# Alfredu/dislib

Measured on AMD Instinct MI355X. Metric: KMeans samples·iters/sec at 1/2/4/8 GPUs + % of HBM/MFMA roofline, higher is better.
Workload: dtype f64

## Files before the change

### dislib_amd/csrc/dkm_dense.h

```cpp
#pragma once

#include <hip/hip_runtime.h>

#include "dkm_internal.h"

namespace dkm {

constexpr int BLOCK = 256;
constexpr size_t LDS_BUDGET = 80 * 1024;
constexpr size_t LDS_PER_CU = 160 * 1024;

enum : int { AM_NONE = 0, AM_ON = 1, AM_DELTA = 2, AM_INLDS = 4,
             AM_MLIST = 8 };
__host__ __device__ __forceinline__ bool am_full(int m) {
  return (m & (AM_ON | AM_DELTA)) == AM_ON;
}

struct DevInfo {
  int cus = 256;
};
DevInfo dev_info();
int resident_blocks(const void *kf, int block, size_t lds);

template <class TX>
__device__ __forceinline__ double ld_x(const TX *p) {
  return (double)(*p);
}

__host__ __device__ __forceinline__ int lds_stride(int d) {
  return (d & 1) ? d : d + 1;
}
__host__ __device__ __forceinline__ int64_t lds_acc_len(int64_t k, int d) {
  return k * lds_stride(d) + k;
}

__device__ __forceinline__ void lds_add(double *p, double v) {
  __hip_atomic_fetch_add(p, v, __ATOMIC_RELAXED, __HIP_MEMORY_SCOPE_WORKGROUP);
}

struct AccTarget {
  double *rows;
  double *cnt;
  int stride;
  bool lds;
  __device__ __forceinline__ void add(int row, int t, double v) const {
    double *p = rows + (int64_t)row * stride + t;
    if (lds)
      lds_add(p, v);
    else
      atomic_add_f64(p, v);
  }
  __device__ __forceinline__ void count(int row, double v) const {
    if (lds)
      lds_add(cnt + row, v);
    else
      atomic_add_f64(cnt + row, v);
  }
};

__device__ __forceinline__ AccTarget acc_target(int amode, double *lds_acc,
                                                double *acc, int64_t k,
                                                int d) {
  if (amode & AM_INLDS) {
    const int ds = lds_stride(d);
    return AccTarget{lds_acc, lds_acc + k * ds, ds, true};
  }
  return AccTarget{acc, acc + k * d, d, false};
}

__device__ __forceinline__ void zero_lds_acc(double *lds_acc, int64_t k,
                                             int d) {
  const int64_t len = lds_acc_len(k, d);
  for (int64_t e = threadIdx.x; e < len; e += blockDim.x) lds_acc[e] = 0.0;
}

__device__ __forceinline__ void flush_lds_acc(const double *lds_acc,
                                              double *acc, int64_t k, int d) {
  const int ds = lds_stride(d);
  const int64_t kd = k * d;
  for (int64_t e = threadIdx.x; e < kd + k; e += blockDim.x) {
    const double v = e < kd ? lds_acc[(e / d) * ds + (e % d)]
                            : lds_acc[k * ds + (e - kd)];
    if (v != 0.0) atomic_add_f64(acc + e, v);
  }
}

template <bool VEC, class TX>
__device__ __forceinline__ void load8(const TX *xr, int t0, int d,
                                      double (&o)[8]) {
  if (VEC) {
    if (t0 < d) {
      if constexpr (sizeof(TX) == 8) {
        const double2 *p = (const double2 *)(xr + t0);
        const double2 a = p[0], b = p[1], c = p[2], e = p[3];
        o[0] = a.x; o[1] = a.y; o[2] = b.x; o[3] = b.y;
        o[4] = c.x; o[5] = c.y; o[6] = e.x; o[7] = e.y;
      } else {
        const float4 *p = (const float4 *)(xr + t0);
        const float4 a = p[0], b = p[1];
        o[0] = a.x; o[1] = a.y; o[2] = a.z; o[3] = a.w;
        o[4] = b.x; o[5] = b.y; o[6] = b.z; o[7] = b.w;
      }
    } else {
#pragma unroll
      for (int m = 0; m < 8; ++m) o[m] = 0.0;
    }
  } else {
#pragma unroll
    for (int m = 0; m < 8; ++m)
      o[m] = (t0 + m < d) ? (double)xr[t0 + m] : 0.0;
  }
}

inline int acc_mode(int acc_kind, bool lds_fits) {
  if (acc_kind == 0) return AM_NONE;
  return AM_ON | (acc_kind == 2 ? AM_DELTA : 0) | (lds_fits ? AM_INLDS : 0);
}

struct RcBnd {
  float *ub, *lb;
};

bool list_ok(int64_t k, int64_t d);
template <class TX>
int launch_list(const TX *X, int d, int64_t ldx, int k, const WsView &v,
                int32_t *lab_out, double *acc, int acc_kind, bool vec,
                int64_t base, int nseg, hipStream_t s, bool wave_all = false,
                const RcBnd *bnd = nullptr);
template <class TX>
int launch_recheck(const TX *X, int64_t end, int d, int64_t ldx, int k,
                   const WsView &v, int32_t *lab_out, double *acc,
                   int acc_kind, bool vec, int64_t base, hipStream_t s,
                   const RcBnd *bnd = nullptr);

}
```

### dislib_amd/csrc/dkm_recheck.hip

```cpp
#include <hip/hip_runtime.h>

#include <algorithm>
#include <cmath>

#include "dkm_dense.h"
#include "dkm_screen.h"

namespace dkm {

__device__ __forceinline__ void wave_lds_sync() {
  __builtin_amdgcn_fence(__ATOMIC_SEQ_CST, "wavefront");
  __builtin_amdgcn_wave_barrier();
}

template <bool UP>
__device__ __forceinline__ float f32_outward(double v) {
  float f = (float)v;
  if (UP) {
    if ((double)f < v) f = __uint_as_float(__float_as_uint(f) + 1u);
  } else {
    if ((double)f > v) f = __uint_as_float(__float_as_uint(f) - 1u);
  }
  return f;
}
__device__ __forceinline__ void settle_bounds(float xx, float b1, float b2,
                                              float B, float *ub, float *lb) {
  const double u2 = fma((double)xx, 1.0 + 0x1.0p-18, (double)b1 + (double)B);
  const double l2 = fma((double)xx, 1.0 - 0x1.0p-18, (double)b2 - (double)B);
  *ub = f32_outward<true>(sqrt(fmax(u2, 0.0)));
  *lb = f32_outward<false>(sqrt(fmax(l2, 0.0)));
}
template <int MAXD, bool VEC, class TX, bool STAGE1_ONLY = false,
          bool BND = false>
__device__ __forceinline__ bool resolve_lane(
    const TX *__restrict__ X, int64_t ldx, int d, int k, int64_t i, int prev,
    const float *cl, const float *cnl, int dp, float cm, const double *ct64,
    int32_t *lab_out, int amode, const AccTarget &at, RcBnd rb = RcBnd{},
    unsigned *nset = nullptr) {
  const TX *xr = X + i * ldx;
  float xf[MAXD];
  float xx = 0.f;
#pragma unroll
  for (int b = 0; b < MAXD / 8; ++b) {
    double o[8];
    if (8 * b < d) {
      load8<VEC>(xr, 8 * b, d, o);
    } else {
#pragma unroll
      for (int m = 0; m < 8; ++m) o[m] = 0.0;
    }
#pragma unroll
    for (int m = 0; m < 8; ++m) {
      xf[8 * b + m] = (float)o[m];
      xx = fmaf(xf[8 * b + m], xf[8 * b + m], xx);
    }
  }
  typedef const __attribute__((address_space(4))) float cfloat;
  typedef const __attribute__((address_space(4))) f32x4 cf32x4;
  cfloat *clc = (cfloat *)cl;
  cfloat *cnc = (cfloat *)cnl;
  const bool full = dp == MAXD;
  auto score = [&](int jc) {
    cfloat *cr = clc + (int64_t)jc * dp;
    float dot = 0.f;
    if (full) {
#pragma unroll
      for (int t4 = 0; t4 < MAXD / 4; ++t4) {
        const f32x4 c4 = *(cf32x4 *)(cr + 4 * t4);
        dot = fmaf(xf[4 * t4 + 0], c4.x, dot);
        dot = fmaf(xf[4 * t4 + 1], c4.y, dot);
        dot = fmaf(xf[4 * t4 + 2], c4.z, dot);
        dot = fmaf(xf[4 * t4 + 3], c4.w, dot);
      }
    } else {
#pragma unroll
      for (int t4 = 0; t4 < MAXD / 4; ++t4) {
        if (4 * t4 < dp) {
          const f32x4 c4 = *(cf32x4 *)(cr + 4 * t4);
          dot = fmaf(xf[4 * t4 + 0], c4.x, dot);
          dot = fmaf(xf[4 * t4 + 1], c4.y, dot);
          dot = fmaf(xf[4 * t4 + 2], c4.z, dot);
          dot = fmaf(xf[4 * t4 + 3], c4.w, dot);
        }
      }
    }
    return fmaf(-2.f, dot, cnc[jc]);
  };
  float b1 = INFINITY, b2 = INFINITY;
  int i1 = 0;
#pragma unroll 4
  for (int jc = 0; jc < k; ++jc) {
    const float sc = score(jc);
    i1 = sc < b1 ? jc : i1;
    b2 = __builtin_amdgcn_fmed3f(b1, b2, sc);
    b1 = fminf(b1, sc);
  }
  const float xn = sqrtf(xx) * (1.0f + (d + 4) * 0x1.0p-24f);
  const float B = screen_bound<P_F32>(d, xn, cm, false);
  const bool sane = (xn < 1e18f) && (xn * cm < 1e30f) && (b1 < 1e30f);
  int bi = i1;
  if (!(sane && b2 - b1 > 2.0f * B)) {
    if constexpr (STAGE1_ONLY) return false;
    const float lim = b1 + 2.0f * B;
    double best = INFINITY;
    bi = -1;
#pragma unroll 1
    for (int jc = 0; jc < k; ++jc) {
      if (sane && !(score(jc) <= lim)) continue;
      const SqDiffT<TX> f{xr, ct64 + jc, ct_ld(k)};
      const double dist = argmin_key(sqrt(pw_leaf(f, 0, d)));
      if (dist < best || bi < 0) {
        best = dist;
        bi = jc;
      }
    }
  } else if constexpr (BND) {
    if (b2 < 1e30f) {
      settle_bounds(xx, b1, b2, B, rb.ub + i, rb.lb + i);
      *nset += 1u;
    }
  }
  lab_out[i] = bi;
  if (!(amode & AM_ON)) return true;
  const bool delta = amode & AM_DELTA;
  if (delta && bi == prev) return true;
  const bool sub = delta && prev >= 0;
  for (int t = 0; t < d; ++t) {
    const double x = ld_x(xr + t);
    at.add(bi, t, x);
    if (sub) at.add(prev, t, -x);
  }
  at.count(bi, 1.0);
  if (sub) at.count(prev, -1.0);
  return true;
}

template <class TX>
__device__ __forceinline__ void recheck_accumulate(int amode,
                                                   const AccTarget &at,
                                                   const TX *xr, int d,
                                                   int bi, int prev,
                                                   int lane) {
  if (!(amode & AM_ON)) return;
  const bool delta = amode & AM_DELTA;
  if (delta && bi == prev) return;
  const bool sub = delta && prev >= 0;
  for (int t = lane; t < d; t += 64) {
    const double x = ld_x(xr + t);
    at.add(bi, t, x);
    if (sub) at.add(prev, t, -x);
  }
  if (lane == 0) {
    at.count(bi, 1.0);
    if (sub) at.count(prev, -1.0);
  }
}

__device__ __forceinline__ void recheck_finish_count(
    unsigned long long mine, unsigned long long *blk_count, const WsView &v) {
  if ((threadIdx.x & 63) == 0 && mine)
    __hip_atomic_fetch_add(blk_count, mine, __ATOMIC_RELAXED,
                           __HIP_MEMORY_SCOPE_WORKGROUP);
  __syncthreads();
  if (threadIdx.x == 0 && *blk_count)
    atomicAdd((unsigned long long *)&v.hdr->rechecked_total, *blk_count);
}

__device__ __forceinline__ void recheck_finish_settled(
    unsigned nset, unsigned long long *blk_settled, const WsView &v) {
  if (nset)
    __hip_atomic_fetch_add(blk_settled, (unsigned long long)nset,
                           __ATOMIC_RELAXED, __HIP_MEMORY_SCOPE_WORKGROUP);
  __syncthreads();
  if (threadIdx.x == 0 && *blk_settled)
    atomicAdd((unsigned long long *)&v.hdr->bnd_settled, *blk_settled);
}

template <int MAXD, class TX>
__device__ __forceinline__ void resolve_wave(
    const TX *__restrict__ X, int64_t ldx, int d, int k, int64_t i, int prev,
    const float *cl, const float *cnl, int dp, float cm, const double *ct64,
    int32_t *lab_out, int amode, const AccTarget &at) {
  const int lane = threadIdx.x & 63;
  const TX *xr = X + i * ldx;
  float xf[MAXD];
  float xx = 0.f;
#pragma unroll
  for (int t = 0; t < MAXD; ++t) {
    xf[t] = t < d ? (float)ld_x(xr + t) : 0.f;
    xx = fmaf(xf[t], xf[t], xx);
  }
  auto score = [&](int jc) {
    const f32x4 *cr = (const f32x4 *)(cl + (int64_t)jc * dp);
    f32x4 c4[MAXD / 4];
#pragma unroll
    for (int t4 = 0; t4 < MAXD / 4; ++t4)
      if (4 * t4 < dp) c4[t4] = cr[t4];
    float dot = 0.f;
#pragma unroll
    for (int t4 = 0; t4 < MAXD / 4; ++t4)
      if (4 * t4 < dp) {
        dot = fmaf(xf[4 * t4 + 0], c4[t4].x, dot);
        dot = fmaf(xf[4 * t4 + 1], c4[t4].y, dot);
        dot = fmaf(xf[4 * t4 + 2], c4[t4].z, dot);
        dot = fmaf(xf[4 * t4 + 3], c4[t4].w, dot);
      }
    return fmaf(-2.f, dot, cnl[jc]);
  };
  float b1 = INFINITY, b2 = INFINITY;
  int i1 = INT32_MAX;
#pragma unroll 2
  for (int jc = lane; jc < k; jc += 64) {
    const float sc = score(jc);
    i1 = sc < b1 ? jc : i1;
    b2 = __builtin_amdgcn_fmed3f(b1, b2, sc);
    b1 = fminf(b1, sc);
  }
  for (int off = 1; off < 64; off <<= 1) {
    const float o1 = __shfl_xor(b1, off, 64), o2 = __shfl_xor(b2, off, 64);
    const int oi = __shfl_xor(i1, off, 64);
    const bool tk = (o1 < b1) | ((o1 == b1) & (oi < i1));
    b2 = tk ? fminf(b1, o2) : fminf(b2, o1);
    i1 = tk ? oi : i1;
    b1 = tk ? o1 : b1;
  }
  const float xn = sqrtf(xx) * (1.0f + (d + 4) * 0x1.0p-24f);
  const float B = screen_bound<P_F32>(d, xn, cm, false);
  const bool sane = (xn < 1e18f) && (xn * cm < 1e30f) && (b1 < 1e30f);
  int bi = i1;
  if (!(sane && b2 - b1 > 2.0f * B)) {
    const float lim = b1 + 2.0f * B;
    double best = INFINITY;
    bi = INT32_MAX;
    for (int jc = lane; jc < k; jc += 64) {
      if (sane && !(score(jc) <= lim)) continue;
      const SqDiffT<TX> f{xr, ct64 + jc, ct_ld(k)};
      const double dist = argmin_key(sqrt(pw_leaf(f, 0, d)));
      if (dist < best || bi == INT32_MAX) {
        best = dist;
        bi = jc;
      }
    }
    for (int off = 1; off < 64; off <<= 1) {
      const double ob = __shfl_xor(best, off, 64);
      const int oi = __shfl_xor(bi, off, 64);
      const bool tk = (ob < best) | ((ob == best) & (oi < bi));
      best = tk ? ob : best;
      bi = tk ? oi : bi;
    }
  }
  if (lane == 0) lab_out[i] = bi;
  recheck_accumulate(amode, at, xr, d, bi, prev, lane);
}

constexpr int RL_CAP = 128;

static size_t recheck_lane_lds(int64_t, int64_t) {
  return (size_t)(BLOCK / 64) * RL_CAP * 8;
}

#define RC_BND 0
#include "dkm_recheck_kernels.inc"
#undef RC_BND
#define RC_BND 1
#include "dkm_recheck_kernels.inc"
#undef RC_BND

template <int MAXD, class TX>
__global__ void __launch_bounds__(BLOCK)
    k_recheck_wave(const TX *__restrict__ X, int d, int64_t ldx, int k,
                   WsView v, int32_t *__restrict__ lab_out, double *acc,
                   int amode, int64_t base) {
  const uint32_t cap = (uint32_t)std::min<int64_t>(v.nq / 2, INT32_MAX);
  const uint32_t cnt = min(v.hdr->s2count, cap);
  const int64_t wv = (int64_t)blockIdx.x * (BLOCK / 64) + (threadIdx.x >> 6);
  const int64_t nwv = (int64_t)gridDim.x * (BLOCK / 64);
  if (wv >= cnt) return;
  const int dp = (int)round_up(d, 4);
  const float cm =
      (float)__longlong_as_double((long long)v.hdr->cmax_bits) * 1.000001f;
  const int am = amode & ~AM_INLDS;
  const AccTarget at = acc_target(am, nullptr, acc, k, d);
  const int2 *s2l = (const int2 *)v.smoved;
  for (int64_t r = wv; r < cnt; r += nwv) {
    const int2 it = s2l[r];
    resolve_wave<MAXD, TX>(X, ldx, d, k, base + it.x, it.y, v.c32, v.cn32,
                           dp, cm, v.ct64, lab_out, am, at);
  }
}

template <bool SMALL, class TX>
__global__ void __launch_bounds__(BLOCK)
    k_recheck_exact(const TX *__restrict__ X, int64_t n, int d, int64_t ldx,
                    int k, WsView v, int32_t *__restrict__ lab_out,
                    double *acc, int amode, int64_t base) {
  if (v.hdr->qcount == 0) return;
  extern __shared__ __attribute__((aligned(16))) double smem[];
  double *lds_acc = smem;
  __shared__ unsigned long long blk_count;
  if (threadIdx.x == 0) blk_count = 0;
  if (amode & AM_INLDS) zero_lds_acc(lds_acc, k, d);
  const AccTarget at = acc_target(amode, lds_acc, acc, k, d);
  __syncthreads();
  const int lane = threadIdx.x & 63;
  const int64_t wv = (int64_t)blockIdx.x * (BLOCK / 64) + (threadIdx.x >> 6);
  const int64_t nwv = (int64_t)gridDim.x * (BLOCK / 64);
  unsigned long long mine = 0;
  for (int64_t c0 = base + wv * 64; c0 < n; c0 += nwv * 64) {
    const int64_t li = c0 + lane;
    const int lv = li < n ? lab_out[li] : 0;
    unsigned long long mask = __ballot(lv < 0);
    mine += __popcll(mask);
    while (mask) {
      const int bit = __ffsll((long long)mask) - 1;
      mask &= mask - 1;
      const int64_t i = c0 + bit;
      const int prev = -__shfl(lv, bit, WAVE) - 2;
      const TX *xr = X + i * ldx;
      double best = INFINITY;
      int bi = 0x7fffffff;
      for (int jc = lane; jc < k; jc += 64) {
        const SqDiffT<TX> f{xr, v.ct64 + jc, ct_ld(k)};
        const double dist =
            argmin_key(sqrt(SMALL ? pw_leaf(f, 0, d) : pw_sum(f, d)));
        if (dist < best || bi == 0x7fffffff) {
          best = dist;
          bi = jc;
        }
      }
      wave_argmin(best, bi);
      if (lane == 0) lab_out[i] = bi;
      recheck_accumulate(amode, at, xr, d, bi, prev, lane);
    }
  }
  recheck_finish_count(mine, &blk_count, v);
  if (amode & AM_INLDS) flush_lds_acc(lds_acc, acc, k, d);
}

template <int MAXD, bool VEC, class TX>
static void launch_recheck_lane_t(unsigned g, size_t lds, hipStream_t s,
                                  const TX *X, int64_t end, int d,
                                  int64_t ldx, int k, const WsView &v,
                                  int32_t *lab_out, double *acc, int amode,
                                  int64_t base) {
  k_recheck_lane<MAXD, VEC, TX><<<g, BLOCK, lds, s>>>(X, end, d, ldx, k, v,
                                                       lab_out, acc, amode,
                                                       base);
}

template <int MAXD, class TX>
static const void *recheck_lane_fn(bool vec) {
  return vec ? (const void *)k_recheck_lane<MAXD, true, TX>
             : (const void *)k_recheck_lane<MAXD, false, TX>;
}

template <class TX>
int launch_recheck(const TX *X, int64_t end, int d, int64_t ldx, int k,
                   const WsView &v, int32_t *lab_out, double *acc,
                   int acc_kind, bool vec, int64_t base, hipStream_t s,
                   const RcBnd *bnd) {
  const size_t a_bytes = (size_t)lds_acc_len(k, d) * 8;
  const size_t fb = recheck_lane_lds(k, d);
  const bool lane = d <= 128 && fb <= LDS_BUDGET;
  const int maxd = d <= 32 ? 32 : d <= 64 ? 64 : 128;
  if (bnd && !(lane && maxd == 32))
    return fail(DKM_E_ARG, "exact re-check: bounds need d <= 32");
  const size_t fixed = lane ? fb : 0;
  const int amode = acc_mode(acc_kind, fixed + a_bytes <= LDS_BUDGET);
  const size_t lds = fixed + ((amode & AM_INLDS) ? a_bytes : 0);
  const bool small = d <= 128;
  const void *kf =
      bnd     ? (vec ? (const void *)k_recheck_lane_bnd<32, true, TX>
                     : (const void *)k_recheck_lane_bnd<32, false, TX>)
      : !lane ? (small ? (const void *)k_recheck_exact<true, TX>
                       : (const void *)k_recheck_exact<false, TX>)
      : maxd == 32 ? recheck_lane_fn<32, TX>(vec)
      : maxd == 64 ? recheck_lane_fn<64, TX>(vec)
                   : recheck_lane_fn<128, TX>(vec);
  const int per_cu = resident_blocks(kf, BLOCK, lds);
  const int64_t waves = (end - base + 3 + (lane ? 255 : 63)) / (lane ? 256 : 64);
  const unsigned g = (unsigned)std::max<int64_t>(
      1, std::min<int64_t>((int64_t)dev_info().cus * per_cu,
                           (waves + BLOCK / 64 - 1) / (BLOCK / 64)));
  if (bnd) {
    if (vec)
      k_recheck_lane_bnd<32, true, TX><<<g, BLOCK, lds, s>>>(
          X, end, d, ldx, k, v, lab_out, acc, amode, base, *bnd);
    else
      k_recheck_lane_bnd<32, false, TX><<<g, BLOCK, lds, s>>>(
          X, end, d, ldx, k, v, lab_out, acc, amode, base, *bnd);
  } else if (lane) {
#define DKM_RL(M)                                                            \
  (vec ? launch_recheck_lane_t<M, true, TX>(g, lds, s, X, end, d, ldx, k, v, \
                                            lab_out, acc, amode, base)       \
       : launch_recheck_lane_t<M, false, TX>(g, lds, s, X, end, d, ldx, k,   \
                                             v, lab_out, acc, amode, base))
    if (maxd == 32)
      DKM_RL(32);
    else if (maxd == 64)
      DKM_RL(64);
    else
      DKM_RL(128);
#undef DKM_RL
  } else if (small) {
    k_recheck_exact<true, TX><<<g, BLOCK, lds, s>>>(X, end, d, ldx, k, v,
                                                     lab_out, acc, amode, base);
  } else {
    k_recheck_exact<false, TX><<<g, BLOCK, lds, s>>>(X, end, d, ldx, k, v,
                                                      lab_out, acc, amode, base);
  }
  return check_launch("exact re-check");
}

template <int MAXD, bool VEC, class TX>
static int launch_list_t(const TX *X, int d, int64_t ldx, int k,
                         const WsView &v, int32_t *lab_out, double *acc,
                         int amode, int64_t base, int nseg, size_t lds,
                         hipStream_t s, bool wave_all) {
  const void *kf = (const void *)k_recheck_list<MAXD, VEC, TX>;
  const int per_cu = resident_blocks(kf, BLOCK, lds);
  const int64_t units = (int64_t)nseg * (TL_CAP / 64);
  const int64_t g = std::max<int64_t>(
      1, std::min<int64_t>((int64_t)dev_info().cus * per_cu,
                           (units + BLOCK / 64 - 1) / (BLOCK / 64)));
  if (hipMemsetAsync(&v.hdr->s2count, 0, 4, s) != hipSuccess)
    return fail(DKM_E_LAUNCH, "list re-check: counter reset");
  k_recheck_list<MAXD, VEC, TX><<<(unsigned)g, BLOCK, lds, s>>>(
      X, d, ldx, k, v, lab_out, acc, amode, base, nseg, wave_all ? 1 : 0);
  if (int r = check_launch("list re-check")) return r;
  if (!wave_all) return 0;
  k_recheck_wave<MAXD, TX><<<(unsigned)(dev_info().cus * 4), BLOCK, 0, s>>>(
      X, d, ldx, k, v, lab_out, acc, amode, base);
  return check_launch("list re-check (wave per sample)");
}

template <bool VEC, class TX>
static int launch_list_bnd_t(const TX *X, int d, int64_t ldx, int k,
                             const WsView &v, int32_t *lab_out, double *acc,
                             int amode, int64_t base, int nseg, size_t lds,
                             hipStream_t s, const RcBnd &rb) {
  const void *kf = (const void *)k_recheck_list_bnd<32, VEC, TX>;
  const int per_cu = resident_blocks(kf, BLOCK, lds);
  const int64_t units = (int64_t)nseg * (TL_CAP / 64);
  const int64_t g = std::max<int64_t>(
      1, std::min<int64_t>((int64_t)dev_info().cus * per_cu,
                           (units + BLOCK / 64 - 1) / (BLOCK / 64)));
  if (hipMemsetAsync(&v.hdr->s2count, 0, 4, s) != hipSuccess)
    return fail(DKM_E_LAUNCH, "list re-check: counter reset");
  k_recheck_list_bnd<32, VEC, TX><<<(unsigned)g, BLOCK, lds, s>>>(
      X, d, ldx, k, v, lab_out, acc, amode, base, nseg, 0, rb);
  return check_launch("list re-check (bounds)");
}

bool list_ok(int64_t k, int64_t d) {
  return d <= 128 && recheck_lane_lds(k, d) <= LDS_BUDGET;
}

template <class TX>
int launch_list(const TX *X, int d, int64_t ldx, int k, const WsView &v,
                int32_t *lab_out, double *acc, int acc_kind, bool vec,
                int64_t base, int nseg, hipStream_t s, bool wave_all,
                const RcBnd *bnd) {
  const size_t fb = 0;
  const size_t a_bytes = (size_t)lds_acc_len(k, d) * 8;
  const int amode = acc_mode(acc_kind, fb + a_bytes <= LDS_BUDGET);
  const size_t lds = fb + ((amode & AM_INLDS) ? a_bytes : 0);
  const int maxd = d <= 32 ? 32 : d <= 64 ? 64 : 128;
  if (bnd) {
    if (maxd != 32 || wave_all)
      return fail(DKM_E_ARG, "list re-check: bounds need d <= 32");
    return vec ? launch_list_bnd_t<true, TX>(X, d, ldx, k, v, lab_out, acc,
                                             amode, base, nseg, lds, s, *bnd)
               : launch_list_bnd_t<false, TX>(X, d, ldx, k, v, lab_out, acc,
                                              amode, base, nseg, lds, s,
                                              *bnd);
  }
#define DKM_LL(M)                                                            \
  (vec ? launch_list_t<M, true, TX>(X, d, ldx, k, v, lab_out, acc, amode,    \
                                    base, nseg, lds, s, wave_all)            \
       : launch_list_t<M, false, TX>(X, d, ldx, k, v, lab_out, acc, amode,   \
                                     base, nseg, lds, s, wave_all))
  const int r = maxd == 32 ? DKM_LL(32) : maxd == 64 ? DKM_LL(64) : DKM_LL(128);
#undef DKM_LL
  return r;
}

#define DKM_RECHECK_INST(TX)                                                 \
  template int launch_recheck<TX>(const TX *, int64_t, int, int64_t, int,    \
                                  const WsView &, int32_t *, double *, int,  \
                                  bool, int64_t, hipStream_t,                \
                                  const RcBnd *);                            \
  template int launch_list<TX>(const TX *, int, int64_t, int,                \
                               const WsView &, int32_t *, double *, int,     \
                               bool, int64_t, int, hipStream_t, bool,        \
                               const RcBnd *);
DKM_RECHECK_INST(double)
DKM_RECHECK_INST(float)
#undef DKM_RECHECK_INST

}

namespace dkm {
DKM_TU_FLAGS(recheck, 0)
__global__ void k_tu_recheck() {}
int preload_recheck() {
  hipFuncAttributes a;
  const bool ok =
      hipFuncGetAttributes(&a, (const void *)k_tu_recheck) == hipSuccess;
  return ok ? 0 : 1;
}
}
```

### dislib_amd/csrc/dkm_recheck_kernels.inc

```
#if RC_BND
#define RC_NAME(x) x##_bnd
#define RC_BND_PARAM , RcBnd rb
#else
#define RC_NAME(x) x
#define RC_BND_PARAM
#endif

template <int MAXD, bool VEC, class TX>
__global__ void __launch_bounds__(BLOCK)
    RC_NAME(k_recheck_lane)(const TX *__restrict__ X, int64_t n, int d, int64_t ldx,
                   int k, WsView v, int32_t *__restrict__ lab_out,
                   double *acc, int amode, int64_t base RC_BND_PARAM) {
  if (v.hdr->qcount == 0) return;
  extern __shared__ __attribute__((aligned(16))) double smem[];
  const int dp = (int)round_up(d, 4);
  int64_t *lists = (int64_t *)smem;
  double *lds_acc = (double *)(lists + (BLOCK / 64) * RL_CAP);
  __shared__ unsigned long long blk_count;
  if (threadIdx.x == 0) blk_count = 0;
#if RC_BND
  __shared__ unsigned long long blk_settled;
  unsigned nset = 0;
  if (threadIdx.x == 0) blk_settled = 0;
#endif
  if (amode & AM_INLDS) zero_lds_acc(lds_acc, k, d);
  const float cm =
      (float)__longlong_as_double((long long)v.hdr->cmax_bits) * 1.000001f;
  const AccTarget at = acc_target(amode, lds_acc, acc, k, d);
  __syncthreads();

  const int lane = threadIdx.x & 63;
  int64_t *wl = lists + (threadIdx.x >> 6) * RL_CAP;

  auto resolve = [&](int64_t i) {
#if RC_BND
    resolve_lane<MAXD, VEC, TX, false, true>(X, ldx, d, k, i,
                                             -lab_out[i] - 2, v.c32, v.cn32,
                                             dp, cm, v.ct64, lab_out, amode,
                                             at, rb, &nset);
#else
    resolve_lane<MAXD, VEC, TX>(X, ldx, d, k, i, -lab_out[i] - 2, v.c32,
                                v.cn32, dp,
                                cm, v.ct64, lab_out, amode, at);
#endif
  };

  const int64_t wv = (int64_t)blockIdx.x * (BLOCK / 64) + (threadIdx.x >> 6);
  const int64_t nwv = (int64_t)gridDim.x * (BLOCK / 64);
  const int64_t a0 =
      base - (int64_t)(((uintptr_t)(lab_out + base) >> 2) & 3);
  auto load4 = [&](int64_t c0, int (&o)[4]) {
    const int64_t i0 = c0 + 4 * lane;
    if (i0 >= base && i0 + 3 < n) {
      const int4 q4 = *(const int4 *)(lab_out + i0);
      o[0] = q4.x; o[1] = q4.y; o[2] = q4.z; o[3] = q4.w;
    } else {
#pragma unroll
      for (int c = 0; c < 4; ++c)
        o[c] = (i0 + c >= base && i0 + c < n) ? lab_out[i0 + c] : 0;
    }
  };
  unsigned long long mine = 0;
  int cnt = 0;
  int cur[4] = {0, 0, 0, 0};
  int64_t c0 = a0 + wv * 256;
  if (c0 < n) load4(c0, cur);
  for (; c0 < n; c0 += nwv * 256) {
    int nxt[4] = {0, 0, 0, 0};
    if (c0 + nwv * 256 < n) load4(c0 + nwv * 256, nxt);
#pragma unroll
    for (int c = 0; c < 4; ++c) {
      const unsigned long long mask = __ballot(cur[c] < 0);
      if (cur[c] < 0)
        wl[cnt + __popcll(mask & ((1ull << lane) - 1))] = c0 + 4 * lane + c;
      const int add = __popcll(mask);
      mine += add;
      cnt += add;
      if (cnt >= 64) {
        wave_lds_sync();
        resolve(wl[lane]);
        const int rem = cnt - 64;
        const int64_t tail = lane < rem ? wl[64 + lane] : 0;
        wave_lds_sync();
        if (lane < rem) wl[lane] = tail;
        cnt = rem;
      }
    }
#pragma unroll
    for (int c = 0; c < 4; ++c) cur[c] = nxt[c];
  }
  wave_lds_sync();
  if (lane < cnt) resolve(wl[lane]);
  recheck_finish_count(mine, &blk_count, v);
#if RC_BND
  recheck_finish_settled(nset, &blk_settled, v);
#endif
  if (amode & AM_INLDS) flush_lds_acc(lds_acc, acc, k, d);
}

template <int MAXD, bool VEC, class TX>
__global__ void __launch_bounds__(BLOCK)
    RC_NAME(k_recheck_list)(const TX *__restrict__ X, int d, int64_t ldx, int k,
                   WsView v, int32_t *__restrict__ lab_out, double *acc,
                   int amode, int64_t base, int nseg, int wave_all
                   RC_BND_PARAM) {
  extern __shared__ __attribute__((aligned(16))) double smem[];
  const int dp = (int)round_up(d, 4);
  double *lds_acc = (double *)smem;
  __shared__ unsigned long long blk_count;
  __shared__ int2 dlist[BLOCK / 64][128];
  if (threadIdx.x == 0) blk_count = 0;
#if RC_BND
  __shared__ unsigned long long blk_settled;
  unsigned nset = 0;
  if (threadIdx.x == 0) blk_settled = 0;
#endif
  if (amode & AM_INLDS) zero_lds_acc(lds_acc, k, d);
  const float cm =
      (float)__longlong_as_double((long long)v.hdr->cmax_bits) * 1.000001f;
  const AccTarget at = acc_target(amode, lds_acc, acc, k, d);
  __syncthreads();
  const int lane = threadIdx.x & 63;
  const int64_t wv = (int64_t)blockIdx.x * (BLOCK / 64) + (threadIdx.x >> 6);
  const int64_t nwv = (int64_t)gridDim.x * (BLOCK / 64);
  unsigned long long mine = 0;
  int2 *dl = dlist[threadIdx.x >> 6];
  int dcnt = 0;
  auto stage2 = [&](int2 it) {
    resolve_lane<MAXD, VEC, TX>(X, ldx, d, k, base + it.x, it.y, v.c32,
                                v.cn32, dp,
                                cm, v.ct64, lab_out, amode, at);
  };
  int2 *s2l = (int2 *)v.smoved;
  const uint32_t s2cap = (uint32_t)std::min<int64_t>(v.nq / 2, INT32_MAX);
  for (int64_t L = wv; L < (int64_t)nseg * (TL_CAP / 64); L += nwv) {
    const int64_t sg = L % nseg;
    const int t0 = (int)(L / nseg) * 64;
    const int cnt = v.tcount[sg];
    if (t0 == 0) mine += cnt;
    if (t0 >= cnt) continue;
    const int2 *e = v.tlist + sg * TL_CAP;
    {
      int2 it = make_int2(0, 0);
      bool ok = true;
      if (t0 + lane < cnt) {
        it = e[t0 + lane];
#if RC_BND
        ok = !wave_all &&
             resolve_lane<MAXD, VEC, TX, true, true>(
                 X, ldx, d, k, base + it.x, it.y, v.c32, v.cn32, dp, cm,
                 v.ct64, lab_out, amode, at, rb, &nset);
#else
        ok = !wave_all &&
             resolve_lane<MAXD, VEC, TX, true>(X, ldx, d, k, base + it.x,
                                               it.y, v.c32, v.cn32, dp, cm,
                                               v.ct64, lab_out, amode, at);
#endif
      }
      unsigned long long m = __ballot(!ok);
      if (m && wave_all) {
        uint32_t pos = 0;
        if (lane == 0) pos = atomicAdd(&v.hdr->s2count, (uint32_t)__popcll(m));
        pos = (uint32_t)__shfl((int)pos, 0, 64);
        const uint32_t p = pos + (uint32_t)__popcll(m & ((1ull << lane) - 1));
        if (!ok && p < s2cap) s2l[p] = it;
        m = __ballot(!ok && p >= s2cap);
        ok = ok || p < s2cap;
      }
      if (!ok) dl[dcnt + __popcll(m & ((1ull << lane) - 1))] = it;
      dcnt += __popcll(m);
      if (dcnt >= 64) {
        wave_lds_sync();
        stage2(dl[lane]);
        const int rem = dcnt - 64;
        const int2 tail = lane < rem ? dl[64 + lane] : make_int2(0, 0);
        wave_lds_sync();
        if (lane < rem) dl[lane] = tail;
        dcnt = rem;
      }
    }
  }
  wave_lds_sync();
  if (lane < dcnt) stage2(dl[lane]);
  recheck_finish_count(mine, &blk_count, v);
#if RC_BND
  recheck_finish_settled(nset, &blk_settled, v);
#endif
  if (amode & AM_INLDS) flush_lds_acc(lds_acc, acc, k, d);
}

#undef RC_NAME
#undef RC_BND_PARAM
```

Measured before the change: 81.99 billion.

## Compact recheck list traversal via prefix sums and software-prefetch next row

The recheck-list kernel now builds a block-wide prefix sum of the per-segment list counts in LDS and walks a dense global index space, binary-searching the segment for each entry. Before, it strided over every segment times TL_CAP/64 slot, including empty ones. It also splits row loading from scoring so the next row's X values can be loaded while the current row is resolved (for MAXD<=32), with entries fetched two iterations ahead. The intent is to cut wasted wave iterations on sparse lists and hide load latency. In exchange, every block repeats the prefix scan with several syncthreads, each entry pays a binary search, the extra raw buffer raises register pressure, and LDS use grows.

```diff
diff --git a/dislib_amd/csrc/dkm_dense.h b/dislib_amd/csrc/dkm_dense.h
--- a/dislib_amd/csrc/dkm_dense.h
+++ b/dislib_amd/csrc/dkm_dense.h
@@ -3,6 +3,7 @@
 #include <hip/hip_runtime.h>
 
 #include "dkm_internal.h"
+#include "dkm_listmap.h"
 
 namespace dkm {
 
diff --git a/dislib_amd/csrc/dkm_listmap.h b/dislib_amd/csrc/dkm_listmap.h
--- /dev/null
+++ b/dislib_amd/csrc/dkm_listmap.h
@@ -0,0 +1,39 @@
+#pragma once
+
+#include <cstdint>
+
+#if defined(__HIPCC__)
+#define DKM_LM_HD __host__ __device__
+#else
+#define DKM_LM_HD
+#endif
+
+namespace dkm {
+
+DKM_LM_HD inline int32_t list_len(int32_t count, int32_t cap) {
+  return count < 0 ? 0 : count > cap ? cap : count;
+}
+
+inline void list_prefix(const int32_t *tcount, int nseg, int32_t cap,
+                        int32_t *pre) {
+  int32_t run = 0;
+  for (int s = 0; s < nseg; ++s) {
+    pre[s] = run;
+    run += list_len(tcount[s], cap);
+  }
+  pre[nseg] = run;
+}
+
+DKM_LM_HD inline int list_segment(const int32_t *pre, int nseg, int32_t pos) {
+  int lo = 0, hi = nseg;
+  while (hi - lo > 1) {
+    const int mid = (lo + hi) >> 1;
+    if (pre[mid] <= pos)
+      lo = mid;
+    else
+      hi = mid;
+  }
+  return lo;
+}
+
+}
diff --git a/dislib_amd/csrc/dkm_recheck.hip b/dislib_amd/csrc/dkm_recheck.hip
--- a/dislib_amd/csrc/dkm_recheck.hip
+++ b/dislib_amd/csrc/dkm_recheck.hip
@@ -30,16 +30,9 @@
   *ub = f32_outward<true>(sqrt(fmax(u2, 0.0)));
   *lb = f32_outward<false>(sqrt(fmax(l2, 0.0)));
 }
-template <int MAXD, bool VEC, class TX, bool STAGE1_ONLY = false,
-          bool BND = false>
-__device__ __forceinline__ bool resolve_lane(
-    const TX *__restrict__ X, int64_t ldx, int d, int k, int64_t i, int prev,
-    const float *cl, const float *cnl, int dp, float cm, const double *ct64,
-    int32_t *lab_out, int amode, const AccTarget &at, RcBnd rb = RcBnd{},
-    unsigned *nset = nullptr) {
-  const TX *xr = X + i * ldx;
-  float xf[MAXD];
-  float xx = 0.f;
+template <int MAXD, bool VEC, class TX>
+__device__ __forceinline__ void load_row(const TX *xr, int d,
+                                         double (&raw)[MAXD]) {
 #pragma unroll
   for (int b = 0; b < MAXD / 8; ++b) {
     double o[8];
@@ -50,11 +43,26 @@
       for (int m = 0; m < 8; ++m) o[m] = 0.0;
     }
 #pragma unroll
-    for (int m = 0; m < 8; ++m) {
-      xf[8 * b + m] = (float)o[m];
-      xx = fmaf(xf[8 * b + m], xf[8 * b + m], xx);
-    }
-  }
+    for (int m = 0; m < 8; ++m) raw[8 * b + m] = o[m];
+  }
+}
+template <int MAXD>
+__device__ __forceinline__ void row_to_f32(const double (&raw)[MAXD],
+                                           float (&xf)[MAXD], float *xx_out) {
+  float xx = 0.f;
+#pragma unroll
+  for (int t = 0; t < MAXD; ++t) {
+    xf[t] = (float)raw[t];
+    xx = fmaf(xf[t], xf[t], xx);
+  }
+  *xx_out = xx;
+}
+template <int MAXD, class TX, bool STAGE1_ONLY = false, bool BND = false>
+__device__ __forceinline__ bool resolve_row(
+    const TX *xr, const float (&xf)[MAXD], float xx, int d, int k, int64_t i,
+    int prev, const float *cl, const float *cnl, int dp, float cm,
+    const double *ct64, int32_t *lab_out, int amode, const AccTarget &at,
+    RcBnd rb = RcBnd{}, unsigned *nset = nullptr) {
   typedef const __attribute__((address_space(4))) float cfloat;
   typedef const __attribute__((address_space(4))) f32x4 cf32x4;
   cfloat *clc = (cfloat *)cl;
@@ -134,6 +142,23 @@
   if (sub) at.count(prev, -1.0);
   return true;
 }
+template <int MAXD, bool VEC, class TX, bool STAGE1_ONLY = false,
+          bool BND = false>
+__device__ __forceinline__ bool resolve_lane(
+    const TX *__restrict__ X, int64_t ldx, int d, int k, int64_t i, int prev,
+    const float *cl, const float *cnl, int dp, float cm, const double *ct64,
+    int32_t *lab_out, int amode, const AccTarget &at, RcBnd rb = RcBnd{},
+    unsigned *nset = nullptr) {
+  const TX *xr = X + i * ldx;
+  double raw[MAXD];
+  float xf[MAXD];
+  float xx;
+  load_row<MAXD, VEC, TX>(xr, d, raw);
+  row_to_f32<MAXD>(raw, xf, &xx);
+  return resolve_row<MAXD, TX, STAGE1_ONLY, BND>(xr, xf, xx, d, k, i, prev, cl,
+                                                 cnl, dp, cm, ct64, lab_out,
+                                                 amode, at, rb, nset);
+}
 
 template <class TX>
 __device__ __forceinline__ void recheck_accumulate(int amode,
@@ -255,10 +280,44 @@
 
 constexpr int RL_CAP = 128;
 
+__device__ __forceinline__ void block_list_prefix(
+    const int32_t *__restrict__ tcount, int nseg, int32_t *pre,
+    int32_t *part) {
+  const int t = threadIdx.x;
+  for (int i = t; i < nseg; i += BLOCK) pre[i] = list_len(tcount[i], TL_CAP);
+  __syncthreads();
+  const int per = (nseg + BLOCK - 1) / BLOCK;
+  const int a = min(nseg, t * per), b = min(nseg, a + per);
+  int sum = 0;
+  for (int i = a; i < b; ++i) sum += pre[i];
+  part[t] = sum;
+  __syncthreads();
+  for (int off = 1; off < BLOCK; off <<= 1) {
+    const int o = t >= off ? part[t - off] : 0;
+    __syncthreads();
+    part[t] += o;
+    __syncthreads();
+  }
+  int run = part[t] - sum;
+  for (int i = a; i < b; ++i) {
+    const int c = pre[i];
+    pre[i] = run;
+    run += c;
+  }
+  if (t == BLOCK - 1) pre[nseg] = part[BLOCK - 1];
+}
+
+static size_t list_prefix_lds(int nseg) {
+  return (size_t)round_up((int64_t)(nseg + 1) * 4, 8);
+}
+
 static size_t recheck_lane_lds(int64_t, int64_t) {
   return (size_t)(BLOCK / 64) * RL_CAP * 8;
 }
 
+#ifndef DKM_AB_RC_PREFETCH
+#define DKM_AB_RC_PREFETCH 1
+#endif
 #define RC_BND 0
 #include "dkm_recheck_kernels.inc"
 #undef RC_BND
@@ -461,7 +520,8 @@
                 int32_t *lab_out, double *acc, int acc_kind, bool vec,
                 int64_t base, int nseg, hipStream_t s, bool wave_all,
                 const RcBnd *bnd) {
-  const size_t fb = 0;
+  nseg = std::max(0, std::min(nseg, TL_SEGS));
+  const size_t fb = list_prefix_lds(nseg);
   const size_t a_bytes = (size_t)lds_acc_len(k, d) * 8;
   const int amode = acc_mode(acc_kind, fb + a_bytes <= LDS_BUDGET);
   const size_t lds = fb + ((amode & AM_INLDS) ? a_bytes : 0);
diff --git a/dislib_amd/csrc/dkm_recheck_kernels.inc b/dislib_amd/csrc/dkm_recheck_kernels.inc
--- a/dislib_amd/csrc/dkm_recheck_kernels.inc
+++ b/dislib_amd/csrc/dkm_recheck_kernels.inc
@@ -107,6 +107,9 @@
   extern __shared__ __attribute__((aligned(16))) double smem[];
   const int dp = (int)round_up(d, 4);
   double *lds_acc = (double *)smem;
+  int32_t *pre =
+      (int32_t *)(smem + ((amode & AM_INLDS) ? lds_acc_len(k, d) : 0));
+  __shared__ int32_t part[BLOCK];
   __shared__ unsigned long long blk_count;
   __shared__ int2 dlist[BLOCK / 64][128];
   if (threadIdx.x == 0) blk_count = 0;
@@ -116,6 +119,7 @@
   if (threadIdx.x == 0) blk_settled = 0;
 #endif
   if (amode & AM_INLDS) zero_lds_acc(lds_acc, k, d);
+  block_list_prefix(v.tcount, nseg, pre, part);
   const float cm =
       (float)__longlong_as_double((long long)v.hdr->cmax_bits) * 1.000001f;
   const AccTarget at = acc_target(amode, lds_acc, acc, k, d);
@@ -123,7 +127,8 @@
   const int lane = threadIdx.x & 63;
   const int64_t wv = (int64_t)blockIdx.x * (BLOCK / 64) + (threadIdx.x >> 6);
   const int64_t nwv = (int64_t)gridDim.x * (BLOCK / 64);
-  unsigned long long mine = 0;
+  const int64_t total = pre[nseg];
+  unsigned long long mine = wv == 0 ? (unsigned long long)total : 0;
   int2 *dl = dlist[threadIdx.x >> 6];
   int dcnt = 0;
   auto stage2 = [&](int2 it) {
@@ -133,28 +138,60 @@
   };
   int2 *s2l = (int2 *)v.smoved;
   const uint32_t s2cap = (uint32_t)std::min<int64_t>(v.nq / 2, INT32_MAX);
-  for (int64_t L = wv; L < (int64_t)nseg * (TL_CAP / 64); L += nwv) {
-    const int64_t sg = L % nseg;
-    const int t0 = (int)(L / nseg) * 64;
-    const int cnt = v.tcount[sg];
-    if (t0 == 0) mine += cnt;
-    if (t0 >= cnt) continue;
-    const int2 *e = v.tlist + sg * TL_CAP;
+  auto entry = [&](int64_t b, int2 *it) {
+    const int64_t p = b * 64 + lane;
+    *it = make_int2(0, 0);
+    if (p >= total) return false;
+    const int sg = list_segment(pre, nseg, (int32_t)p);
+    *it = v.tlist[(int64_t)sg * TL_CAP + ((int32_t)p - pre[sg])];
+    return true;
+  };
+  constexpr bool PF = DKM_AB_RC_PREFETCH && MAXD <= 32;
+  double raw[PF ? MAXD : 1];
+  auto rows = [&](bool a, int2 it) {
+    if constexpr (PF) {
+      if (a && !wave_all)
+        load_row<MAXD, VEC, TX>(X + (base + it.x) * ldx, d, raw);
+    }
+  };
+  int64_t b = wv;
+  int2 it1, it2;
+  bool a1 = entry(b, &it1);
+  bool a2 = entry(b + nwv, &it2);
+  rows(a1, it1);
+  for (; b * 64 < total; b += nwv) {
+    const int2 it = it1;
+    const bool act = a1;
+    float xf[MAXD];
+    float xx = 0.f;
+    if constexpr (PF) {
+      if (act && !wave_all) row_to_f32<MAXD>(raw, xf, &xx);
+    }
+    it1 = it2;
+    a1 = a2;
+    rows(a1, it1);
+    a2 = entry(b + 2 * nwv, &it2);
     {
-      int2 it = make_int2(0, 0);
       bool ok = true;
-      if (t0 + lane < cnt) {
-        it = e[t0 + lane];
+      if (act) {
+        const TX *xr = X + (base + it.x) * ldx;
+        if constexpr (!PF) {
+          if (!wave_all) {
+            double r[MAXD];
+            load_row<MAXD, VEC, TX>(xr, d, r);
+            row_to_f32<MAXD>(r, xf, &xx);
+          }
+        }
 #if RC_BND
         ok = !wave_all &&
-             resolve_lane<MAXD, VEC, TX, true, true>(
-                 X, ldx, d, k, base + it.x, it.y, v.c32, v.cn32, dp, cm,
+             resolve_row<MAXD, TX, true, true>(
+                 xr, xf, xx, d, k, base + it.x, it.y, v.c32, v.cn32, dp, cm,
                  v.ct64, lab_out, amode, at, rb, &nset);
 #else
         ok = !wave_all &&
-             resolve_lane<MAXD, VEC, TX, true>(X, ldx, d, k, base + it.x,
-                                               it.y, v.c32, v.cn32, dp, cm,
-                                               v.ct64, lab_out, amode, at);
+             resolve_row<MAXD, TX, true>(xr, xf, xx, d, k, base + it.x, it.y,
+                                         v.c32, v.cn32, dp, cm, v.ct64,
+                                         lab_out, amode, at);
 #endif
       }
       unsigned long long m = __ballot(!ok);
```

Result: slower. 81.05 billion (-1.1%).
